# CouncilmanJeremyJamm/path_tracer

Measured on AMD Instinct MI355X. Metric: Mray/s at 1920x1080, 256 spp; achieved HBM GB/s in traversal kernel, higher is better.
Workload: dtype f32; 1 GPU; Cornell box (36 triangles, 6 BLAS) 1920x1080, 256 spp, depth 8, NEE+MIS; parallelism=rows/1, bvh_in_lds=True, scene_bytes=4208

## Files before the change

### path_tracer_amd/csrc/pt_api.cpp

```cpp
#include "../../include/pt_api.h"

#include <hip/hip_runtime.h>

#include <algorithm>
#include <chrono>
#include <cmath>
#include <cstdio>
#include <cstdlib>
#include <cstring>
#include <mutex>
#include <string>
#include <vector>

#include "pt_kernels.h"
#include "pt_png.h"
#include "pt_scene.h"

using namespace pt;

#ifndef PT_SHADE_BLOCKS_PER_CU
#define PT_SHADE_BLOCKS_PER_CU 16
#endif
#ifndef PT_JOIN_LATE
#define PT_JOIN_LATE 0
// ... 222 lines not shown
    if ((r = up(c->d_materials, f.materials.data(), f.materials.size() * sizeof(DMaterial)))) return r;
    if ((r = up(c->d_lights, f.lights.data(), f.lights.size() * sizeof(DLight)))) return r;

    SceneView& sv = c->sv;
    uint8_t* base = (uint8_t*)c->d_blob.p;
    sv.nodes = (const DNode*)base;
    sv.tri_isect = (const DTriIsect*)(base + nb);
    sv.instances = (const DInstance*)(base + nb + tb);
    sv.tri_shade = (const DTriVerts*)c->d_tri_shade.p;
    sv.tri_pos = (const DTriVerts*)c->d_tri_pos.p;
    sv.tri_orig = (const uint32_t*)c->d_tri_orig.p;
    sv.materials = (const DMaterial*)c->d_materials.p;
    sv.lights = (const DLight*)c->d_lights.p;
    sv.n_nodes = (uint32_t)f.nodes.size();
    sv.n_tris = (uint32_t)f.tri_isect.size();
    sv.n_instances = (uint32_t)f.instances.size();
    sv.n_materials = (uint32_t)f.materials.size();
    sv.n_lights = (uint32_t)f.lights.size();
    sv.world_root = f.world_root;
    sv.lights_root = f.lights_root;
    sv.prim_bits = f.prim_bits;
    sv.light_weight_sum = f.light_weight_sum;
    sv.blob_bytes = (uint32_t)blob.size();
    sv.stack_entries = f.stack_entries;
    sv.has_volumes = f.has_volumes ? 1u : 0u;
    c->ident_tlas = f.ident_tlas;

    c->lds_scene = blob.size() <= 48 * 1024 && !(c->cfg.flags & PT_FLAG_NO_LDS_SCENE);
    uint32_t threads = 256;
#ifndef PT_STACK_LDS_LEVELS
#define PT_STACK_LDS_LEVELS 14
#endif
    sv.stack_lds = std::min<uint32_t>(sv.stack_entries, c->cfg.stack_lds_levels ? c->cfg.stack_lds_levels : PT_STACK_LDS_LEVELS);
    auto lds_need = [&](uint32_t t) { return trace_lds_bytes(c->lds_scene, sv.blob_bytes, sv.stack_lds, t); };
    while (threads > 64 && lds_need(threads) > 64 * 1024) threads >>= 1;
    if (lds_need(threads) > 160 * 1024) return fail(c, PT_ERR_LIMIT, "BVH too deep for the LDS traversal stack");
    c->block_threads = threads;
    const size_t lds = lds_need(threads);
    uint32_t per_cu = (uint32_t)std::min<size_t>((160 * 1024) / std::max<size_t>(lds, 1), 2048 / threads);
    per_cu = std::max(1u, std::min(per_cu, (uint32_t)PT_TRACE_BLOCKS_PER_CU_MAX));
    c->trace_blocks = (uint32_t)c->n_cus * per_cu;
    sv.stack_spill = nullptr;
    if (sv.stack_entries > sv.stack_lds)
    {
        const size_t lanes = (size_t)c->trace_blocks * threads;
        c->spill_region_words = (size_t)(sv.stack_entries - sv.stack_lds) * lanes;
        if ((r = dev_alloc(c, c->d_spill, 2 * pt_ctx::kMaxPipes * c->spill_region_words * 8))) return r;
        sv.stack_spill = (uint64_t*)c->d_spill.p;
    }

    for (uint32_t q = 0; q < Q_COUNT; ++q) c->class_present[q] = (q == Q_TERMINAL);
    for (const DInstance& in : f.instances) c->class_present[in.qclass & 0xffu] = true;
    c->scene_uploaded = true;
    c->stats.scene_bytes = blob.size();
    c->stats.lds_scene = c->lds_scene;
    c->stats.stack_entries = sv.stack_entries;
    return PT_OK;
}

TraceLaunch trace_launch(pt_ctx* c, int pipe = 0, bool side_stream = false)
{
    TraceLaunch tl;
    tl.scene = c->sv;
    if (tl.scene.stack_spill) tl.scene.stack_spill += (size_t)(2 * pipe + (side_stream ? 1 : 0)) * c->spill_region_words;
    tl.blob = c->d_blob.p;
    tl.lds_scene = c->lds_scene;
    tl.ident_tlas = (c->cfg.flags & PT_FLAG_GENERAL_WALK) ? 0u : c->ident_tlas;
// ... 1967 lines not shown
```

### path_tracer_amd/csrc/pt_kernels.h

```cpp
#pragma once
#include <hip/hip_runtime.h>

#include "pt_materials.h"
#include "pt_types.h"

namespace pt {

struct TraceLaunch
{
    SceneView scene;
    const void* blob;
    bool lds_scene;
    uint32_t ident_tlas;
    uint32_t grid_blocks;
    uint32_t n_cus;
    uint32_t block_threads;
};

inline size_t trace_lds_bytes(bool lds_scene, uint32_t blob_bytes, uint32_t stack_lds, uint32_t block_threads)
{
    return (lds_scene ? (size_t)blob_bytes : 0) + (size_t)stack_lds * block_threads * 8;
}
inline size_t trace_lds_bytes(const TraceLaunch& tl) { return trace_lds_bytes(tl.lds_scene, tl.scene.blob_bytes, tl.scene.stack_lds, tl.block_threads); }

struct WavefrontBuffers
{
    PathState st;
    RayQueue rq[2];
    RayQueue rq_shadow;
    RayQueue rq_lchain[2];
    f4* lchain_nb[2];
    f4* lchain_hit;
    f4* hits;
    f4* q_shade_base;
    uint32_t q_stride;
    uint32_t q_class_slot;
    uint2* q_term[2];
    Counters* counters;
    uint32_t* heads;
    uint4* wave_times;
    uint4* wave_times_any;
    uint32_t* tails;
    uint32_t cap_slots;
    uint32_t cap_slots_shade;
    uint32_t cap_slots_term;
    uint32_t class_mask;
};

inline ShadeQueue shade_queue(const WavefrontBuffers& wb, uint32_t q)
{
    const size_t slot = (wb.q_class_slot >> (4u * q)) & 0xfu;
    f4* a = wb.q_shade_base + 3u * slot * (size_t)wb.q_stride;
    return ShadeQueue{a, a + wb.q_stride, a + 2u * (size_t)wb.q_stride};
}

void launch_generate(hipStream_t s, const RenderParams& rp, const CameraView& cam, const WavefrontBuffers& wb, const uint2* list = nullptr);
// ... 35 lines not shown
```

### path_tracer_amd/csrc/pt_kernels.hip

```cpp
#include "pt_kernels.h"
#include "pt_materials.h"

#include <algorithm>
#include <mutex>
#include <vector>

namespace pt {
namespace {

#ifndef PT_STEPS_PER_ROUND
#define PT_STEPS_PER_ROUND 8
#endif
#ifndef PT_REFILL_BELOW
#define PT_REFILL_BELOW 40
#endif
#ifndef PT_STEPS_PER_ROUND_GLOBAL_BVH
#define PT_STEPS_PER_ROUND_GLOBAL_BVH 4
#endif
#ifndef PT_REFILL_BELOW_GLOBAL_BVH
#define PT_REFILL_BELOW_GLOBAL_BVH 56
#endif
#ifndef PT_STEPS_ANY
#define PT_STEPS_ANY 4
#endif
// ... 366 lines not shown
            else base = nb;
        }
        sh.base[q] = base;
    }
    __syncthreads();
#pragma unroll
    for (int q = 0; q < 4; ++q) pos[q] = sh.base[q] + sh.wave_rank[q][wid] + mbcnt64(m[q]);
    __syncthreads();
}

__device__ __forceinline__ f3 xyz(const f4& v) { return f3{v.x, v.y, v.z}; }
__device__ __forceinline__ float asf(uint32_t u) { return __uint_as_float(u); }
__device__ __forceinline__ uint32_t asu(float f) { return __float_as_uint(f); }

typedef float nt4_t __attribute__((ext_vector_type(4)));
__device__ __forceinline__ void nt_store(f4* p, f4 v) { __builtin_nontemporal_store(nt4_t{v.x, v.y, v.z, v.w}, reinterpret_cast<nt4_t*>(p)); }
__device__ __forceinline__ f4 nt_load(const f4* p) { const nt4_t v = __builtin_nontemporal_load(reinterpret_cast<const nt4_t*>(p)); return f4{v.x, v.y, v.z, v.w}; }


__device__ __forceinline__ bool slab(const uint4 w0, const uint4 w1, const f3 o, const f3 inv, const float t_max, float& t_enter)
{
    const bool nx = inv.x < 0.0f, ny = inv.y < 0.0f, nz = inv.z < 0.0f;
    typedef float pair_t __attribute__((ext_vector_type(2)));
    const pair_t px = (pair_t{asf(nx ? w1.x : w0.x), asf(nx ? w0.x : w1.x)} - pair_t{o.x, o.x}) * pair_t{inv.x, inv.x};
    const pair_t py = (pair_t{asf(ny ? w1.y : w0.y), asf(ny ? w0.y : w1.y)} - pair_t{o.y, o.y}) * pair_t{inv.y, inv.y};
    const pair_t pz = (pair_t{asf(nz ? w1.z : w0.z), asf(nz ? w0.z : w1.z)} - pair_t{o.z, o.z}) * pair_t{inv.z, inv.z};
    const float tnx = px.x, tfx = px.y, tny = py.x, tfy = py.y, tnz = pz.x, tfz = pz.y;
    const float ts = fmaxf(fmaxf(fmaxf(tnx, tny), tnz), PT_EPSILON);
    const float tb = fminf(fminf(fminf(tfx, tfy), tfz), t_max);
    t_enter = ts;
    return ts <= tb;
}

__device__ __forceinline__ bool sign_differs(float a, float b)
{
    return __builtin_isunordered(a, b) || (((asu(a) ^ asu(b)) >> 31) != 0u);
}

__device__ __forceinline__ bool tri_planes(const uint4 p0, const uint4 p1, const uint4 p2, const f3 o, const f3 d, const float t_max,
                                           const float t_est, float& td, float& ud, float& vd, float& det)
{
    const f3 mo = fma3(d, bc3(t_est), o);
    const float t_min = PT_EPSILON - t_est, t_mx = t_max - t_est;
    const f4 n0{asf(p0.x), asf(p0.y), asf(p0.z), asf(p0.w)};
    det = dot3(d, xyz(n0));
    td = -dot4(f4{mo.x, mo.y, mo.z, -1.0f}, n0);
    const bool out_t = sign_differs(td - det * t_min, det * t_mx - td);
    const f3 p = det * mo + td * d;
    const f4 p4{p.x, p.y, p.z, det};
    ud = dot4(p4, f4{asf(p1.x), asf(p1.y), asf(p1.z), asf(p1.w)});
    const bool out_u = sign_differs(ud, det - ud);
    vd = dot4(p4, f4{asf(p2.x), asf(p2.y), asf(p2.z), asf(p2.w)});
    const bool out_v = sign_differs(vd, det - ud - vd);
    return !(out_t | out_u | out_v);
}

struct TriEval { float td, ud, vd, det; bool uv_ok; };
__device__ __forceinline__ TriEval tri_eval(const uint4* tp, const f3 mo, const f3 d)
{
    TriEval e;
    const uint4 p0 = tp[0], p1 = tp[1], p2 = tp[2];
    const f4 n0{asf(p0.x), asf(p0.y), asf(p0.z), asf(p0.w)};
    e.det = dot3(d, xyz(n0));
    e.td = -dot4(f4{mo.x, mo.y, mo.z, -1.0f}, n0);
    const f3 p = e.det * mo + e.td * d;
    const f4 p4{p.x, p.y, p.z, e.det};
    e.ud = dot4(p4, f4{asf(p1.x), asf(p1.y), asf(p1.z), asf(p1.w)});
    e.vd = dot4(p4, f4{asf(p2.x), asf(p2.y), asf(p2.z), asf(p2.w)});
    const bool out_u = sign_differs(e.ud, e.det - e.ud), out_v = sign_differs(e.vd, e.det - e.ud - e.vd);
    e.uv_ok = !out_u && !out_v;
    return e;
}
__device__ __forceinline__ bool tri_in_range(const TriEval& e, float t_min, float t_mx) { return !sign_differs(e.td - e.det * t_min, e.det * t_mx - e.td); }

struct Blob
{
    const uint4* nodes;
    const uint4* tris;
    const uint4* inst;
    const uint2* leaves;
};
__device__ __forceinline__ void leaf_range(const Blob& bl, uint32_t kind, uint32_t payload, uint32_t& first, uint32_t& count)
{
    if (kind == NODE_TRIS) { first = payload & LEAF_FIRST_MASK; count = (payload >> LEAF_FIRST_BITS) + 1u; }
    else { const uint2 lf = bl.leaves[payload]; first = lf.x; count = lf.y; }
}

struct LaneRay { f3 o, d, inv; };

__device__ __forceinline__ void pin(uint4& v) { asm volatile("" : "+v"(v.x), "+v"(v.y), "+v"(v.z), "+v"(v.w)); }
template <bool EAGER, bool ROOT_BOX>
__device__ __forceinline__ LaneRay to_object(const Blob& bl, uint32_t inst, const LaneRay& w, bool ray_finite, uint4& root0, uint4& root1)
{
    const uint4* ip = bl.inst + INST_WORDS * inst;
    uint4 r0, r1, r2;
    if (EAGER)
    {
        r0 = ip[0]; r1 = ip[1]; r2 = ip[2];
    }
    const uint4 meta = ip[INST_META_WORD];
    if (ROOT_BOX) { root0 = ip[INST_ROOT_WORD]; root1 = ip[INST_ROOT_WORD + 1u]; }
    else root0.w = reinterpret_cast<const uint32_t*>(ip + INST_ROOT_WORD)[3];
    if (EAGER) { pin(r0); pin(r1); pin(r2); }
    LaneRay r;
    if ((meta.w & INSTANCE_IDENTITY) != 0u && ray_finite)
    {
        const uint32_t so = asu(w.o.x) & asu(w.o.y) & asu(w.o.z) & 0x80000000u;
        const uint32_t sd = asu(w.d.x) & asu(w.d.y) & asu(w.d.z) & 0x80000000u;
        r.o.x = w.o.x != 0.0f ? w.o.x : asf(so);
        r.o.y = w.o.y != 0.0f ? w.o.y : asf(so);
        r.o.z = w.o.z != 0.0f ? w.o.z : asf(so);
        r.d.x = w.d.x != 0.0f ? w.d.x : asf(sd);
        r.d.y = w.d.y != 0.0f ? w.d.y : asf(sd);
        r.d.z = w.d.z != 0.0f ? w.d.z : asf(sd);
        r.inv.x = w.d.x != 0.0f ? w.inv.x : asf(sd | 0x7f800000u);
        r.inv.y = w.d.y != 0.0f ? w.inv.y : asf(sd | 0x7f800000u);
        r.inv.z = w.d.z != 0.0f ? w.inv.z : asf(sd | 0x7f800000u);
        return r;
    }
// ... 3 lines not shown
    r.o.z = ((asf(r2.x) * w.o.x + asf(r2.y) * w.o.y) + asf(r2.z) * w.o.z) + asf(r2.w);
    r.d.x = (asf(r0.x) * w.d.x + asf(r0.y) * w.d.y) + asf(r0.z) * w.d.z;
    r.d.y = (asf(r1.x) * w.d.x + asf(r1.y) * w.d.y) + asf(r1.z) * w.d.z;
    r.d.z = (asf(r2.x) * w.d.x + asf(r2.y) * w.d.y) + asf(r2.z) * w.d.z;
    r.inv = rcp3(r.d);
    return r;
}

__device__ __forceinline__ LaneRay ident_ray(const LaneRay& w)
{
    const uint32_t so = asu(w.o.x) & asu(w.o.y) & asu(w.o.z) & 0x80000000u;
    const uint32_t sd = asu(w.d.x) & asu(w.d.y) & asu(w.d.z) & 0x80000000u;
    LaneRay r;
    r.o.x = w.o.x != 0.0f ? w.o.x : asf(so);
    r.o.y = w.o.y != 0.0f ? w.o.y : asf(so);
    r.o.z = w.o.z != 0.0f ? w.o.z : asf(so);
    r.d.x = w.d.x != 0.0f ? w.d.x : asf(sd);
    r.d.y = w.d.y != 0.0f ? w.d.y : asf(sd);
    r.d.z = w.d.z != 0.0f ? w.d.z : asf(sd);
    r.inv = w.inv;
    return r;
}
__device__ __forceinline__ uint32_t ray_signs(const LaneRay& w)
{
    return (asu(w.o.x) >> 31) | ((asu(w.o.y) >> 31) << 1) | ((asu(w.o.z) >> 31) << 2) |
           ((asu(w.d.x) >> 31) << 3) | ((asu(w.d.y) >> 31) << 4) | ((asu(w.d.z) >> 31) << 5);
}
__device__ __forceinline__ f3 with_signs(const f3 v, uint32_t bits)
{
    return f3{asf((asu(v.x) & 0x7fffffffu) | ((bits & 1u) << 31)), asf((asu(v.y) & 0x7fffffffu) | (((bits >> 1) & 1u) << 31)),
              asf((asu(v.z) & 0x7fffffffu) | (((bits >> 2) & 1u) << 31))};
}

template <bool LDS_SCENE>
__device__ __forceinline__ Blob stage_scene(const SceneView& sv, const uint4* __restrict__ gblob, uint4* smem, uint32_t& words)
{
    Blob b;
    const uint4* base = gblob;
    words = 0;
    if (LDS_SCENE)
    {
        words = sv.blob_bytes >> 4;
        for (uint32_t i = threadIdx.x; i < words; i += blockDim.x) smem[i] = gblob[i];
        __syncthreads();
        base = smem;
    }
    b.nodes = base;
    b.tris = base + 2u * sv.n_nodes;
    b.inst = base + 2u * sv.n_nodes + 3u * sv.n_tris;
    b.leaves = reinterpret_cast<const uint2*>(base + 2u * sv.n_nodes + 3u * sv.n_tris + INST_WORDS * sv.n_instances);
    return b;
}

enum { CLOSEST_WORLD = 0, CLOSEST_LIGHTS = 1, CLOSEST_HOOK = 2, CLOSEST_PRIMARY = 3 };

struct ClosestOut
{
    f4* hits;
    f4* q_base;
    uint32_t q_stride, q_class_slot;
    uint2* q_term;
    uint32_t* n_shade;
    uint4* wave_times;
    uint32_t* tails;
    uint32_t cap_shade, cap_term;
    uint32_t class_mask;
    uint32_t* overflow;
    uint32_t world_root;
    uint8_t* occl;
    f3 eye;
    f4* radiance;
    f4* first_pos;
    uint32_t* first_id;
    uint32_t keep_s_id, keep_s_pos, blk_log, n_blk, blk_last, act_pixels;
    FastDiv div_blk_paths, div_blk_last;
    uint32_t finalize_miss;
    const DPathRec* rec;
    uint32_t enable_nee;
};

template <bool SPILL>
struct Stack8;
template <>
// ... 229 lines not shown
            if (!active && rank < take)
            {
                const uint32_t mine = first + rank;
                const f4 b = rb[mine];
                ray_idx = mine;
                pid = asu(b.w);
                if (pid != HOLE) {
                valid_rays += 1u;
                if (MODE == CLOSEST_PRIMARY)
                {
                    w.o = f3{out->eye.x, out->eye.y, out->eye.z};
                    t_max = asf(0x7f800000u);
                }
                else
                {
                    const f4 a = ra[mine];
                    w.o = xyz(a);
                    t_max = a.w;
                }
                w.d = xyz(b);
                w.inv = rcp3(w.d);
                ray_finite = finite3(w.o) && finite3(w.d);
                if (IDENT) { ob = ident_ray(w); w_signs = ray_signs(w); }
                bid = MISS_ID;
                any_phase = false;
                chain_code = 2u;
                bt = asf(0x7f800000u);
                hud = 0.0f;
                hvd = 0.0f;
                hdet = 1.0f;
                in_blas = false;
                sp = stk.empty();
                float te;
                const uint4 root0 = bl.nodes[2u * root];
                const bool ok = (t_max == t_max) && (!IDENT || ray_finite) && slab(root0, bl.nodes[2u * root + 1u], IDENT ? ob.o : w.o, w.inv, t_max, te);
                if (ok)
                {
                    stk.put(sp, make_uint2(root0.w, 0u));
                    sp = stk.up(sp);
                    active = true;
                }
                else { pending = true; }
                }
            }
#if PT_WAVE_TIMES
            if (tw_first == 0u && take != 0u) tw_first = (uint32_t)wall_clock64() | 1u;
#endif
            act = __ballot(active);
            if (act == 0ull) continue;
            if (PT_RESERVICE && take < (uint32_t)__popcll(idle) && !wr.drained && (uint32_t)__popcll(act) <= (uint32_t)Refill<LDS_SCENE>::kBelow) continue;
        }

#pragma unroll 1
        for (int it = 0; it < Refill<LDS_SCENE>::kSteps; ++it)
        {
#if PT_STEP_STATS
            {
                const uint64_t am = __ballot(active);
                if (am != 0ull) { st_iter += 1u; st_lane_active += (uint32_t)__popcll(am); }
            }
#endif
            if (!active) continue;
            if (!IDENT && in_blas && sp == blas_base) in_blas = false;
            if (MODE == CLOSEST_LIGHTS && any_phase)
            {
                if (sp == stk.empty()) { active = false; pending = true; chain_code = 0u; continue; }
                sp = stk.down(sp);
                const uint2 e = stk.get(sp);
                uint32_t link = e.x;
                float t_enter = asf(e.y);
                if ((link >> NODE_KIND_SHIFT) == NODE_INSTANCE)
                {
                    uint4 r0, r1;
                    if (IDENT)
                    {
                        const uint4* ip = bl.inst + INST_WORDS * (link & NODE_PAYLOAD_MASK) + INST_ROOT_WORD;
                        r0 = ip[0]; r1 = ip[1];
                    }
                    else
                    {
                        ob = to_object<!LDS_SCENE, true>(bl, link & NODE_PAYLOAD_MASK, w, ray_finite, r0, r1);
                        in_blas = true;
                        blas_base = sp;
                    }
                    if (!slab(r0, r1, ob.o, ob.inv, t_max, t_enter)) continue;
                    link = r0.w;
                }
                const uint32_t kkind = link >> NODE_KIND_SHIFT, kpay = link & NODE_PAYLOAD_MASK;
                if (kkind == NODE_BRANCH)
                {
                    const uint4* cp = bl.nodes + 2u * kpay;
                    const uint4 l0 = cp[0], l1 = cp[1], r0 = cp[2], r1 = cp[3];
                    const f3 so = (IDENT || in_blas) ? ob.o : w.o, sinv = (IDENT || in_blas) ? ob.inv : w.inv;
                    float tl, tr;
                    const bool hl = slab(l0, l1, so, sinv, t_max, tl);
                    const bool hr = slab(r0, r1, so, sinv, t_max, tr);
                    if (hl) { stk.put(sp, make_uint2(l0.w, asu(tl))); sp = stk.up(sp); }
                    if (hr) { stk.put(sp, make_uint2(r0.w, asu(tr))); sp = stk.up(sp); }
                }
                else
                {
                    uint32_t first, count;
                    leaf_range(bl, kkind, kpay, first, count);
                    for (uint32_t k = 0; k < count; ++k)
                    {
                        const uint4* tp = bl.tris + 3u * (first + k);
                        float td, ud, vd, det;
                        if (tri_planes(tp[0], tp[1], tp[2], ob.o, ob.d, t_max, t_enter, td, ud, vd, det))
                        {
                            active = false;
                            pending = true;
                            chain_code = 1u;
                            break;
                        }
                    }
                }
                continue;
            }
            if (sp == stk.empty())
            {
                if (MODE == CLOSEST_LIGHTS && bid != MISS_ID)
                {
                    light_hits += 1u;
                    any_phase = true;
                    in_blas = false;
                    t_max = bt * (1.0f - PT_EPSILON);
                    float te = 0.0f;
                    const uint4 wr0 = bl.nodes[2u * lights_world_root];
                    if (t_max == t_max && slab(wr0, bl.nodes[2u * lights_world_root + 1u], IDENT ? ob.o : w.o, IDENT ? ob.inv : w.inv, t_max, te)) { stk.put(sp, make_uint2(wr0.w, asu(te))); sp = stk.up(sp); }
                    else { active = false; pending = true; chain_code = 0u; }
                    continue;
                }
                active = false;
                pending = true;
                continue;
            }
            sp = stk.down(sp);
            const uint2 e = stk.get(sp);
            if (asf(e.y) > t_max) continue;
            uint32_t link = e.x;
            float t_est = asf(e.y);
#if PT_STEP_STATS
            { const bool x = (link >> NODE_KIND_SHIFT) == NODE_INSTANCE; const uint64_t m = __ballot(x); st_lane_inst += x ? 1u : 0u; if (m != 0ull && lane_id() == (uint32_t)__builtin_ctzll(m)) st_wave_inst += 1u; }
#endif
            if ((link >> NODE_KIND_SHIFT) == NODE_INSTANCE)
            {
                uint4 root0, root1;
                inst = link & NODE_PAYLOAD_MASK;
                if (IDENT) root0.w = reinterpret_cast<const uint32_t*>(bl.inst + INST_WORDS * inst + INST_ROOT_WORD)[3];
                else
                {
                    ob = to_object<!LDS_SCENE, false>(bl, inst, w, ray_finite, root0, root1);
                    in_blas = true;
                    blas_base = sp;
                }
                if (0.0f > t_max) continue;
                link = root0.w;
                t_est = 0.0f;
            }
            uint32_t kind = link >> NODE_KIND_SHIFT, payload = link & NODE_PAYLOAD_MASK;
#if PT_STEP_STATS
            { const bool x = kind == NODE_BRANCH; const uint64_t m = __ballot(x); st_lane_branch += x ? 1u : 0u; if (m != 0ull && lane_id() == (uint32_t)__builtin_ctzll(m)) st_wave_branch += 1u; }
#endif
#pragma unroll 1
            for (int lvl = 0; lvl < PT_BRANCH_LEVELS && kind == NODE_BRANCH; ++lvl)
            {
                const uint4* cp = bl.nodes + 2u * payload;
                const uint4 l0 = cp[0], l1 = cp[1], r0 = cp[2], r1 = cp[3];
                const f3 o = (IDENT || in_blas) ? ob.o : w.o, inv = (IDENT || in_blas) ? ob.inv : w.inv;
                float tl, tr;
                const bool hl = slab(l0, l1, o, inv, t_max, tl);
                const bool hr = slab(r0, r1, o, inv, t_max, tr);
                const bool left_near = tl < tr;
                const uint2 le = make_uint2(l0.w, asu(tl)), re = make_uint2(r0.w, asu(tr));
                if (hl && hr) { stk.put(sp, left_near ? re : le); sp = stk.up(sp); }
                kind = NODE_INSTANCE;
                if (hl || hr)
                {
                    const uint2 near = (hl && (left_near || !hr)) ? le : re;
                    const uint32_t nk = near.x >> NODE_KIND_SHIFT;
                    if ((nk & 1u) != 0u || (nk == NODE_BRANCH && lvl + 1 < PT_BRANCH_LEVELS))
                    {
                        kind = nk;
                        payload = near.x & NODE_PAYLOAD_MASK;
                        t_est = asf(near.y);
                    }
                    else { stk.put(sp, near); sp = stk.up(sp); }
                }
            }
#if PT_STEP_STATS
            { const bool x = (kind & 1u) != 0u; const uint64_t m = __ballot(x); st_lane_leaf += x ? 1u : 0u; if (m != 0ull && lane_id() == (uint32_t)__builtin_ctzll(m)) st_wave_leaf += 1u; }
#endif
            if (kind & 1u)
            {
                uint32_t first, count;
                leaf_range(bl, kind, payload, first, count);
                const f3 mo = fma3(ob.d, bc3(t_est), ob.o);
                const float t_min = PT_EPSILON - t_est;
                auto accept = [&](const TriEval& e, uint32_t tri) {
                    if (e.uv_ok && tri_in_range(e, t_min, t_max - t_est))
                    {
                        bt = e.td / e.det + t_est;
                        hud = e.ud;
                        hvd = e.vd;
                        hdet = e.det;
                        t_max = bt;
                        bid = (inst << prim_bits) | tri;
// ... 105 lines not shown
    for (;;)
    {
        uint64_t act = __ballot(active);
        const bool no_more = wr.drained && wr.cur >= wr.end;
#if PT_WAVE_TIMES
        if (no_more && tw_drained == 0u) tw_drained = (uint32_t)wall_clock64() | 1u;
#endif
        const bool service = no_more ? (act == 0ull) : (__popcll(act) <= Refill<LDS_SCENE>::kBelowAny);
        if (service)
        {
            if (no_more) break;
            const uint64_t idle = ~act;
            uint32_t first;
            const uint32_t take = claim_rays(wr, heads, plan, (uint32_t)__popcll(idle), first);
            const uint32_t rank = mbcnt64(idle);
            if (!active && rank < take)
            {
                const uint32_t mine = first + rank;
                const f4 a = ra[mine], b = rb[mine];
                const uint32_t tag = asu(b.w);
                if (tag != HOLE) {
                valid_rays += 1u;
                path_ends = MODE == ANY_SHADOW && (tag & PATH_ENDS) != 0u;
                out_idx = (MODE == ANY_HOOK) ? mine : (tag & ~PATH_ENDS);
                w.o = xyz(a);
                w.d = xyz(b);
                w.inv = rcp3(w.d);
                ray_finite = finite3(w.o) && finite3(w.d);
                if (IDENT) ob = ident_ray(w);
                t_max = a.w;
                in_blas = false;
                sp = stk.empty();
                float te;
                const uint4 root0 = bl.nodes[2u * root];
                const bool ok = (t_max == t_max) && (!IDENT || ray_finite) && slab(root0, bl.nodes[2u * root + 1u], IDENT ? ob.o : w.o, w.inv, t_max, te);
                if (ok)
                {
                    stk.put(sp, make_uint2(root0.w, asu(te)));
                    sp = stk.up(sp);
                    active = true;
                }
                else put_result(0u);
                }
            }
            act = __ballot(active);
            if (act == 0ull) continue;
            if (PT_RESERVICE && take < (uint32_t)__popcll(idle) && !wr.drained && (uint32_t)__popcll(act) <= (uint32_t)Refill<LDS_SCENE>::kBelowAny) continue;
        }

#pragma unroll 1
        for (int it = 0; it < Refill<LDS_SCENE>::kStepsAny; ++it)
        {
#if PT_STEP_STATS
            {
                const uint64_t am = __ballot(active);
                if (am != 0ull) { st_iter += 1u; st_lane_active += (uint32_t)__popcll(am); }
            }
#endif
            if (!active) continue;
            if (!IDENT && in_blas && sp == blas_base) in_blas = false;
            if (sp == stk.empty())
            {
                active = false;
                put_result(0u);
                continue;
            }
            sp = stk.down(sp);
            const uint2 e = stk.get(sp);
            uint32_t link = e.x;
            float t_enter = asf(e.y);
#if PT_STEP_STATS
            { const bool x = (link >> NODE_KIND_SHIFT) == NODE_INSTANCE; const uint64_t m = __ballot(x); st_lane_inst += x ? 1u : 0u; if (m != 0ull && lane_id() == (uint32_t)__builtin_ctzll(m)) st_wave_inst += 1u; }
#endif
            if ((link >> NODE_KIND_SHIFT) == NODE_INSTANCE)
            {
                uint4 r0, r1;
                if (IDENT)
                {
                    const uint4* ip = bl.inst + INST_WORDS * (link & NODE_PAYLOAD_MASK) + INST_ROOT_WORD;
                    r0 = ip[0]; r1 = ip[1];
                }
                else
                {
                    ob = to_object<!LDS_SCENE, true>(bl, link & NODE_PAYLOAD_MASK, w, ray_finite, r0, r1);
                    in_blas = true;
                    blas_base = sp;
                }
                if (!slab(r0, r1, ob.o, ob.inv, t_max, t_enter)) continue;
                link = r0.w;
            }
            uint32_t kind = link >> NODE_KIND_SHIFT, payload = link & NODE_PAYLOAD_MASK;
#if PT_STEP_STATS
            { const bool x = kind == NODE_BRANCH; const uint64_t m = __ballot(x); st_lane_branch += x ? 1u : 0u; if (m != 0ull && lane_id() == (uint32_t)__builtin_ctzll(m)) st_wave_branch += 1u; }
#endif
#pragma unroll 1
            for (int lvl = 0; lvl < PT_BRANCH_LEVELS_ANY && kind == NODE_BRANCH; ++lvl)
            {
                const uint4* cp = bl.nodes + 2u * payload;
                const uint4 l0 = cp[0], l1 = cp[1], r0 = cp[2], r1 = cp[3];
                const f3 o = (IDENT || in_blas) ? ob.o : w.o, inv = (IDENT || in_blas) ? ob.inv : w.inv;
                float tl, tr;
                const bool hl = slab(l0, l1, o, inv, t_max, tl);
                const bool hr = slab(r0, r1, o, inv, t_max, tr);
                if (hl && hr) { stk.put(sp, make_uint2(l0.w, asu(tl))); sp = stk.up(sp); }
                kind = NODE_INSTANCE;
                if (hl || hr)
                {
                    const uint2 next = hr ? make_uint2(r0.w, asu(tr)) : make_uint2(l0.w, asu(tl));
                    const uint32_t nk = next.x >> NODE_KIND_SHIFT;
                    if ((nk & 1u) != 0u || (nk == NODE_BRANCH && lvl + 1 < PT_BRANCH_LEVELS_ANY))
                    {
                        kind = nk;
                        payload = next.x & NODE_PAYLOAD_MASK;
                        t_enter = asf(next.y);
                    }
                    else { stk.put(sp, next); sp = stk.up(sp); }
                }
            }
#if PT_STEP_STATS
            { const bool x = (kind & 1u) != 0u; const uint64_t m = __ballot(x); st_lane_leaf += x ? 1u : 0u; if (m != 0ull && lane_id() == (uint32_t)__builtin_ctzll(m)) st_wave_leaf += 1u; }
#endif
            if (kind & 1u)
            {
                uint32_t first, count;
                leaf_range(bl, kind, payload, first, count);
                for (uint32_t k = 0; k < count; ++k)
                {
                    const uint4* tp = bl.tris + 3u * (first + k);
                    float td, ud, vd, det;
                    if (tri_planes(tp[0], tp[1], tp[2], ob.o, ob.d, t_max, t_enter, td, ud, vd, det))
                    {
                        active = false;
                        put_result(1u);
                        break;
                    }
                }
            }
        }
    }
#if PT_STEP_STATS
    if (MODE == ANY_SHADOW)
// ... 281 lines not shown
                {
                    const PidParts pp = pid_split(rp, pid);
                    if (pp.s == rp.keep_s_pos)
                    {
                        const f3 p = fma3(xyz(rb), bc3(hit.x), xyz(ra));
                        io.st.first_pos[pp.k] = f4{p.x, p.y, p.z, hit.x};
                    }
                    if (pp.s >= rp.keep_s_id) io.st.first_id[(pp.s - rp.keep_s_id) * rp.act_pixels + pp.k] = in.blas & 0xffu;
                }
                const DMaterial& m = sv.materials[in.material];
                if (!rp.enable_nee || (flags & FLAG_LAST_DELTA) || bounce == 0u)
                    acc = fma3(f3{m.colour[0], m.colour[1], m.colour[2]}, pw, acc);
            }
        }
        io.st.radiance[pid] = f4{acc.x, acc.y, acc.z, 0.0f};
    }
}

template <bool IDENT>
__device__ __forceinline__ bool inline_any(const Blob& bl, const Stack8<false>& stk, const uint32_t root, const f4 ra, const f4 rb, const bool want)
{
    bool active = false, blocked = false, in_blas = false, ray_finite = false;
    LaneRay w{}, ob{};
    const float t_max = ra.w;
    uint32_t sp = stk.empty(), blas_base = 0u;
    if (want)
    {
        w.o = xyz(ra);
        w.d = xyz(rb);
        w.inv = rcp3(w.d);
        ray_finite = finite3(w.o) && finite3(w.d);
        if (IDENT) ob = ident_ray(w);
        float te;
        const uint4 root0 = bl.nodes[2u * root];
        if ((t_max == t_max) && (!IDENT || ray_finite) && slab(root0, bl.nodes[2u * root + 1u], IDENT ? ob.o : w.o, w.inv, t_max, te))
        {
            stk.put(sp, make_uint2(root0.w, asu(te)));
            sp = stk.up(sp);
            active = true;
        }
    }
    while (__ballot(active) != 0ull)
    {
        if (!active) continue;
        if (!IDENT && in_blas && sp == blas_base) in_blas = false;
        if (sp == stk.empty()) { active = false; continue; }
        sp = stk.down(sp);
        const uint2 e = stk.get(sp);
        uint32_t link = e.x;
        float t_enter = asf(e.y);
        if ((link >> NODE_KIND_SHIFT) == NODE_INSTANCE)
        {
            uint4 r0, r1;
            if (IDENT)
            {
                const uint4* ip = bl.inst + INST_WORDS * (link & NODE_PAYLOAD_MASK) + INST_ROOT_WORD;
                r0 = ip[0]; r1 = ip[1];
            }
            else
            {
                ob = to_object<false, true>(bl, link & NODE_PAYLOAD_MASK, w, ray_finite, r0, r1);
                in_blas = true;
                blas_base = sp;
            }
            if (!slab(r0, r1, ob.o, ob.inv, t_max, t_enter)) continue;
            link = r0.w;
        }
        uint32_t kind = link >> NODE_KIND_SHIFT, payload = link & NODE_PAYLOAD_MASK;
#pragma unroll 1
        for (int lvl = 0; lvl < PT_BRANCH_LEVELS_INLINE && kind == NODE_BRANCH; ++lvl)
        {
            const uint4* cp = bl.nodes + 2u * payload;
            const uint4 l0 = cp[0], l1 = cp[1], r0 = cp[2], r1 = cp[3];
            const f3 o = (IDENT || in_blas) ? ob.o : w.o, inv = (IDENT || in_blas) ? ob.inv : w.inv;
            float tl, tr;
            const bool hl = slab(l0, l1, o, inv, t_max, tl);
            const bool hr = slab(r0, r1, o, inv, t_max, tr);
            if (hl && hr) { stk.put(sp, make_uint2(l0.w, asu(tl))); sp = stk.up(sp); }
            kind = NODE_INSTANCE;
            if (hl || hr)
            {
                const uint2 next = hr ? make_uint2(r0.w, asu(tr)) : make_uint2(l0.w, asu(tl));
                const uint32_t nk = next.x >> NODE_KIND_SHIFT;
                if ((nk & 1u) != 0u || (nk == NODE_BRANCH && lvl + 1 < PT_BRANCH_LEVELS_INLINE))
                {
                    kind = nk;
                    payload = next.x & NODE_PAYLOAD_MASK;
                    t_enter = asf(next.y);
                }
                else { stk.put(sp, next); sp = stk.up(sp); }
            }
        }
        if (kind & 1u)
        {
            uint32_t first, count;
            leaf_range(bl, kind, payload, first, count);
            for (uint32_t k = 0; k < count; ++k)
            {
                const uint4* tp = bl.tris + 3u * (first + k);
                float td, ud, vd, det;
                if (tri_planes(tp[0], tp[1], tp[2], ob.o, ob.d, t_max, t_enter, td, ud, vd, det))
                {
                    active = false;
                    blocked = true;
                    break;
                }
            }
        }
    }
    return blocked;
}

struct ShadeKArgs { SceneView sv; RenderParams rp; ShadeIO io; uint32_t bounce; const uint4* gblob; uint32_t world_root; };
typedef const __attribute__((address_space(4))) ShadeKArgs* ShadeKArgsPtr;
__device__ __forceinline__ const ShadeKArgs& shade_args()
// ... 286 lines not shown
        if (want_lchain) { io.rq_lchain.a[pos[1]] = lc_a; io.rq_lchain.b[pos[1]] = lc_b; io.lchain_nb[pos[1]] = nee_b; nee_e.w = asf(pos[1]); }
        if (want_next) { nt_store(io.rq_out.a + pos[2], nx_a); nt_store(io.rq_out.b + pos[2], nx_b); }
        if (want_dead) io.q_term_next[pos[3]] = make_uint2(pid | ENTRY_DEAD, pid);
        const bool write_rec = valid && (want_next || want_dead || ends_with_shadow);
        if (valid && !write_rec) io.st.radiance[pid] = f4{acc.x, acc.y, acc.z, 0.0f};
        {
            float m[4][4] = {{pw.x, pw.y, pw.z, asf(draws)}, {acc.x, acc.y, acc.z, asf(flags)}, {nee_e.x, nee_e.y, nee_e.z, nee_e.w}, {nee_pw.x, nee_pw.y, nee_pw.z, nee_pw.w}};
            const uint32_t q = threadIdx.x & 3u;
#pragma unroll
            for (int c = 0; c < 4; ++c)
            {
                float a0 = m[0][c], a1 = m[1][c], a2 = m[2][c], a3 = m[3][c];
                { const float t = (q & 1u) ? a0 : a1; const float r = asf(__builtin_amdgcn_mov_dpp(asu(t), 0xB1, 0xF, 0xF, true)); if (q & 1u) a0 = r; else a1 = r; }
                { const float t = (q & 1u) ? a2 : a3; const float r = asf(__builtin_amdgcn_mov_dpp(asu(t), 0xB1, 0xF, 0xF, true)); if (q & 1u) a2 = r; else a3 = r; }
                { const float t = (q & 2u) ? a0 : a2; const float r = asf(__builtin_amdgcn_mov_dpp(asu(t), 0x4E, 0xF, 0xF, true)); if (q & 2u) a0 = r; else a2 = r; }
                { const float t = (q & 2u) ? a1 : a3; const float r = asf(__builtin_amdgcn_mov_dpp(asu(t), 0x4E, 0xF, 0xF, true)); if (q & 2u) a1 = r; else a3 = r; }
                m[0][c] = a0; m[1][c] = a1; m[2][c] = a2; m[3][c] = a3;
            }
            const uint32_t wr = write_rec ? 1u : 0u;
#define PT_QUAD_STORE(K, SEL)                                                                                                   \
            {                                                                                                                      \
                const uint32_t pid_k = __builtin_amdgcn_mov_dpp(pid, SEL, 0xF, 0xF, true);                \
                const uint32_t wr_k = __builtin_amdgcn_mov_dpp(wr, SEL, 0xF, 0xF, true);                                           \
                if (wr_k != 0u) reinterpret_cast<f4*>(io.st.rec + pid_k)[q] = f4{m[K][0], m[K][1], m[K][2], m[K][3]};             \
            }
            PT_QUAD_STORE(0, 0x00) PT_QUAD_STORE(1, 0x55) PT_QUAD_STORE(2, 0xAA) PT_QUAD_STORE(3, 0xFF)
#undef PT_QUAD_STORE
        }
        if (INLINE)
        {
            uint32_t tid = threadIdx.x;
            asm volatile("" : "+v"(tid));
            const ShadeKArgs& ka2 = shade_args();
            const uint32_t blob_words = ka2.sv.blob_bytes >> 4;
            Blob bl;
            bl.nodes = smem_dyn;
            bl.tris = smem_dyn + 2u * ka2.sv.n_nodes;
            bl.inst = smem_dyn + 2u * ka2.sv.n_nodes + 3u * ka2.sv.n_tris;
            bl.leaves = reinterpret_cast<const uint2*>(smem_dyn + 2u * ka2.sv.n_nodes + 3u * ka2.sv.n_tris + INST_WORDS * ka2.sv.n_instances);
            const Stack8<false> stk{reinterpret_cast<char*>(smem_dyn), blob_words * 16u + tid * 8u, blockDim.x * 8u};
            traced += (uint32_t)__popcll(__ballot(want_shadow));
            culled += (uint32_t)__popcll(__ballot(cull_now));
            const bool blocked = inline_any<IDENT>(bl, stk, ka2.world_root, sh_a, sh_b, want_shadow);
            if (want_shadow)
            {
                DPathRec* rec = shade_args().io.st.rec + pid;
                if (ends_with_shadow)
                {
                    const f3 e = blocked ? f3{0.0f, 0.0f, 0.0f} : xyz(rec->nee_e);
                    const f3 a2 = xyz(rec->acc) + xyz(rec->nee_pw) * (e + f3{0.0f, 0.0f, 0.0f});
                    shade_args().io.st.radiance[pid] = f4{a2.x, a2.y, a2.z, 0.0f};
                }
                else if (blocked)
                {
                    float* e = reinterpret_cast<float*>(&rec->nee_e);
                    e[0] = 0.0f; e[1] = 0.0f; e[2] = 0.0f;
                }
            }
            a_next = (idx + stride) < n ? nt_load(shade_args().io.q_in.a + idx + stride) : hole_a;
        }
    }
    if (!INLINE) add_tally(io.lchain_heads, culled, HEAD_TALLY2);
    else if (lane_id() == 0u)
    {
        const uint32_t wave = blockIdx.x * (blockDim.x >> 6) + (threadIdx.x >> 6);
        const uint32_t line = ((wave * 7u) & (kQueueHeads - 1u)) * kHeadStrideWords;
        if (culled != 0u) atomicAdd(io.lchain_heads + line + HEAD_TALLY2, culled);
        if (traced != 0u) atomicAdd(io.shadow_heads + line + HEAD_TALLY0, traced);
    }
}

#undef PT_SHADE_ARGS
// ... 630 lines not shown
```

Measured before the change: 14730 Mray/s.

## Repack LDS BVH nodes into sign-indexed slab records for branchless child tests

When the scene is staged in LDS, BVH nodes are rewritten into a 10-dword record per node laid out as (min,max,min) triplets per axis plus a link word. The ray's direction sign picks an offset into each triplet, so near/far slab values are read directly and no min/max swap is needed per axis. The goal is fewer ALU ops and narrower LDS reads per child test. In exchange LDS staging gets more complex, node storage grows from 8 to 10 dwords, and accesses become scalar dword loads instead of 128-bit loads, which could add LDS instructions.

Result: faster. 14940 Mray/s, median of 6 (+1.4%).

```diff
diff --git a/path_tracer_amd/csrc/pt_api.cpp b/path_tracer_amd/csrc/pt_api.cpp
--- a/path_tracer_amd/csrc/pt_api.cpp
+++ b/path_tracer_amd/csrc/pt_api.cpp
@@ -278,7 +278,7 @@
 #define PT_STACK_LDS_LEVELS 14
 #endif
     sv.stack_lds = std::min<uint32_t>(sv.stack_entries, c->cfg.stack_lds_levels ? c->cfg.stack_lds_levels : PT_STACK_LDS_LEVELS);
-    auto lds_need = [&](uint32_t t) { return trace_lds_bytes(c->lds_scene, sv.blob_bytes, sv.stack_lds, t); };
+    auto lds_need = [&](uint32_t t) { return trace_lds_bytes(c->lds_scene, sv.blob_bytes, sv.n_nodes, sv.stack_lds, t); };
     while (threads > 64 && lds_need(threads) > 64 * 1024) threads >>= 1;
     if (lds_need(threads) > 160 * 1024) return fail(c, PT_ERR_LIMIT, "BVH too deep for the LDS traversal stack");
     c->block_threads = threads;
diff --git a/path_tracer_amd/csrc/pt_kernels.h b/path_tracer_amd/csrc/pt_kernels.h
--- a/path_tracer_amd/csrc/pt_kernels.h
+++ b/path_tracer_amd/csrc/pt_kernels.h
@@ -17,11 +17,15 @@
     uint32_t block_threads;
 };
 
-inline size_t trace_lds_bytes(bool lds_scene, uint32_t blob_bytes, uint32_t stack_lds, uint32_t block_threads)
+enum : uint32_t { LDS_NODE_DWORDS = 10u, LDS_NODE_LINK = 9u };
+__host__ __device__ inline uint32_t lds_node_words(uint32_t n_nodes) { return (n_nodes * LDS_NODE_DWORDS * 4u + 15u) >> 4; }
+__host__ __device__ inline uint32_t lds_blob_bytes(uint32_t blob_bytes, uint32_t n_nodes) { return blob_bytes - n_nodes * (uint32_t)sizeof(DNode) + lds_node_words(n_nodes) * 16u; }
+
+inline size_t trace_lds_bytes(bool lds_scene, uint32_t blob_bytes, uint32_t n_nodes, uint32_t stack_lds, uint32_t block_threads)
 {
-    return (lds_scene ? (size_t)blob_bytes : 0) + (size_t)stack_lds * block_threads * 8;
+    return (lds_scene ? (size_t)lds_blob_bytes(blob_bytes, n_nodes) : 0) + (size_t)stack_lds * block_threads * 8;
 }
-inline size_t trace_lds_bytes(const TraceLaunch& tl) { return trace_lds_bytes(tl.lds_scene, tl.scene.blob_bytes, tl.scene.stack_lds, tl.block_threads); }
+inline size_t trace_lds_bytes(const TraceLaunch& tl) { return trace_lds_bytes(tl.lds_scene, tl.scene.blob_bytes, tl.scene.n_nodes, tl.scene.stack_lds, tl.block_threads); }
 
 struct WavefrontBuffers
 {
diff --git a/path_tracer_amd/csrc/pt_kernels.hip b/path_tracer_amd/csrc/pt_kernels.hip
--- a/path_tracer_amd/csrc/pt_kernels.hip
+++ b/path_tracer_amd/csrc/pt_kernels.hip
@@ -422,6 +422,25 @@
     return ts <= tb;
 }
 
+struct SlabOff { uint32_t x, y, z; };
+__device__ __forceinline__ SlabOff slab_off(const f3 inv) { return SlabOff{inv.x < 0.0f ? 4u : 0u, inv.y < 0.0f ? 4u : 0u, inv.z < 0.0f ? 4u : 0u}; }
+__device__ __forceinline__ bool slab_lds(const uint32_t* rec, const SlabOff so, const f3 o, const f3 inv, const float t_max, float& t_enter)
+{
+    const char* r = reinterpret_cast<const char*>(rec);
+    const float* ax = reinterpret_cast<const float*>(r + so.x);
+    const float* ay = reinterpret_cast<const float*>(r + so.y) + 3;
+    const float* az = reinterpret_cast<const float*>(r + so.z) + 6;
+    typedef float pair_t __attribute__((ext_vector_type(2)));
+    const pair_t px = (pair_t{ax[0], ax[1]} - pair_t{o.x, o.x}) * pair_t{inv.x, inv.x};
+    const pair_t py = (pair_t{ay[0], ay[1]} - pair_t{o.y, o.y}) * pair_t{inv.y, inv.y};
+    const pair_t pz = (pair_t{az[0], az[1]} - pair_t{o.z, o.z}) * pair_t{inv.z, inv.z};
+    const float tnx = px.x, tfx = px.y, tny = py.x, tfy = py.y, tnz = pz.x, tfz = pz.y;
+    const float ts = fmaxf(fmaxf(fmaxf(tnx, tny), tnz), PT_EPSILON);
+    const float tb = fminf(fminf(fminf(tfx, tfy), tfz), t_max);
+    t_enter = ts;
+    return ts <= tb;
+}
+
 __device__ __forceinline__ bool sign_differs(float a, float b)
 {
     return __builtin_isunordered(a, b) || (((asu(a) ^ asu(b)) >> 31) != 0u);
@@ -466,6 +485,7 @@
 struct Blob
 {
     const uint4* nodes;
+    const uint32_t* lnodes;
     const uint4* tris;
     const uint4* inst;
     const uint2* leaves;
@@ -475,6 +495,31 @@
     if (kind == NODE_TRIS) { first = payload & LEAF_FIRST_MASK; count = (payload >> LEAF_FIRST_BITS) + 1u; }
     else { const uint2 lf = bl.leaves[payload]; first = lf.x; count = lf.y; }
 }
+template <bool LDS_SCENE>
+__device__ __forceinline__ void test_children(const Blob& bl, const uint32_t payload, const f3 o, const f3 inv, const float t_max,
+                                              bool& hl, bool& hr, float& tl, float& tr, uint32_t& ll, uint32_t& lr)
+{
+    if (LDS_SCENE)
+    {
+        const uint32_t* rec = reinterpret_cast<const uint32_t*>(reinterpret_cast<const char*>(bl.lnodes) + __umul24(payload, LDS_NODE_DWORDS * 4u));
+        const SlabOff so = slab_off(inv);
+        hl = slab_lds(rec, so, o, inv, t_max, tl);
+        hr = slab_lds(rec + LDS_NODE_DWORDS, so, o, inv, t_max, tr);
+        ll = rec[LDS_NODE_LINK];
+        lr = rec[LDS_NODE_DWORDS + LDS_NODE_LINK];
+    }
+    else
+    {
+        const uint4* cp = bl.nodes + 2u * payload;
+        const uint4 l0 = cp[0], l1 = cp[1], r0 = cp[2], r1 = cp[3];
+        hl = slab(l0, l1, o, inv, t_max, tl);
+        hr = slab(r0, r1, o, inv, t_max, tr);
+        ll = l0.w;
+        lr = r0.w;
+    }
+}
+__device__ __forceinline__ uint4 lds_box0(const Blob& bl, uint32_t i) { const uint32_t* r = bl.lnodes + LDS_NODE_DWORDS * i; return make_uint4(r[0], r[3], r[6], r[LDS_NODE_LINK]); }
+__device__ __forceinline__ uint4 lds_box1(const Blob& bl, uint32_t i) { const uint32_t* r = bl.lnodes + LDS_NODE_DWORDS * i; return make_uint4(r[1], r[4], r[7], 0u); }
 
 struct LaneRay { f3 o, d, inv; };
 
@@ -544,23 +589,46 @@
               asf((asu(v.z) & 0x7fffffffu) | (((bits >> 2) & 1u) << 31))};
 }
 
+__device__ __forceinline__ Blob lds_blob(uint4* smem, uint32_t blob_bytes, uint32_t n_nodes, uint32_t n_tris, uint32_t n_instances, uint32_t& words)
+{
+    const uint32_t nw = lds_node_words(n_nodes);
+    Blob b;
+    b.nodes = nullptr;
+    b.lnodes = reinterpret_cast<const uint32_t*>(smem);
+    b.tris = smem + nw;
+    b.inst = smem + nw + 3u * n_tris;
+    b.leaves = reinterpret_cast<const uint2*>(smem + nw + 3u * n_tris + INST_WORDS * n_instances);
+    words = nw + (blob_bytes >> 4) - 2u * n_nodes;
+    return b;
+}
 template <bool LDS_SCENE>
 __device__ __forceinline__ Blob stage_scene(const SceneView& sv, const uint4* __restrict__ gblob, uint4* smem, uint32_t& words)
 {
     Blob b;
-    const uint4* base = gblob;
     words = 0;
     if (LDS_SCENE)
     {
-        words = sv.blob_bytes >> 4;
-        for (uint32_t i = threadIdx.x; i < words; i += blockDim.x) smem[i] = gblob[i];
+        b = lds_blob(smem, sv.blob_bytes, sv.n_nodes, sv.n_tris, sv.n_instances, words);
+        const uint32_t nw = lds_node_words(sv.n_nodes), rest = (sv.blob_bytes >> 4) - 2u * sv.n_nodes;
+        for (uint32_t i = threadIdx.x; i < rest; i += blockDim.x) smem[nw + i] = gblob[2u * sv.n_nodes + i];
+        uint32_t* rec = reinterpret_cast<uint32_t*>(smem);
+        for (uint32_t i = threadIdx.x; i < sv.n_nodes; i += blockDim.x)
+        {
+            const uint4 a = gblob[2u * i], m = gblob[2u * i + 1u];
+            uint32_t* r = rec + LDS_NODE_DWORDS * i;
+            r[0] = a.x; r[1] = m.x; r[2] = a.x;
+            r[3] = a.y; r[4] = m.y; r[5] = a.y;
+            r[6] = a.z; r[7] = m.z; r[8] = a.z;
+            r[LDS_NODE_LINK] = a.w;
+        }
         __syncthreads();
-        base = smem;
-    }
-    b.nodes = base;
-    b.tris = base + 2u * sv.n_nodes;
-    b.inst = base + 2u * sv.n_nodes + 3u * sv.n_tris;
-    b.leaves = reinterpret_cast<const uint2*>(base + 2u * sv.n_nodes + 3u * sv.n_tris + INST_WORDS * sv.n_instances);
+        return b;
+    }
+    b.nodes = gblob;
+    b.lnodes = nullptr;
+    b.tris = gblob + 2u * sv.n_nodes;
+    b.inst = gblob + 2u * sv.n_nodes + 3u * sv.n_tris;
+    b.leaves = reinterpret_cast<const uint2*>(gblob + 2u * sv.n_nodes + 3u * sv.n_tris + INST_WORDS * sv.n_instances);
     return b;
 }
 
@@ -856,8 +924,8 @@
                 in_blas = false;
                 sp = stk.empty();
                 float te;
-                const uint4 root0 = bl.nodes[2u * root];
-                const bool ok = (t_max == t_max) && (!IDENT || ray_finite) && slab(root0, bl.nodes[2u * root + 1u], IDENT ? ob.o : w.o, w.inv, t_max, te);
+                const uint4 root0 = LDS_SCENE ? lds_box0(bl, root) : bl.nodes[2u * root];
+                const bool ok = (t_max == t_max) && (!IDENT || ray_finite) && slab(root0, LDS_SCENE ? lds_box1(bl, root) : bl.nodes[2u * root + 1u], IDENT ? ob.o : w.o, w.inv, t_max, te);
                 if (ok)
                 {
                     stk.put(sp, make_uint2(root0.w, 0u));
@@ -913,14 +981,13 @@
                 const uint32_t kkind = link >> NODE_KIND_SHIFT, kpay = link & NODE_PAYLOAD_MASK;
                 if (kkind == NODE_BRANCH)
                 {
-                    const uint4* cp = bl.nodes + 2u * kpay;
-                    const uint4 l0 = cp[0], l1 = cp[1], r0 = cp[2], r1 = cp[3];
                     const f3 so = (IDENT || in_blas) ? ob.o : w.o, sinv = (IDENT || in_blas) ? ob.inv : w.inv;
                     float tl, tr;
-                    const bool hl = slab(l0, l1, so, sinv, t_max, tl);
-                    const bool hr = slab(r0, r1, so, sinv, t_max, tr);
-                    if (hl) { stk.put(sp, make_uint2(l0.w, asu(tl))); sp = stk.up(sp); }
-                    if (hr) { stk.put(sp, make_uint2(r0.w, asu(tr))); sp = stk.up(sp); }
+                    bool hl, hr;
+                    uint32_t ll, lr;
+                    test_children<LDS_SCENE>(bl, kpay, so, sinv, t_max, hl, hr, tl, tr, ll, lr);
+                    if (hl) { stk.put(sp, make_uint2(ll, asu(tl))); sp = stk.up(sp); }
+                    if (hr) { stk.put(sp, make_uint2(lr, asu(tr))); sp = stk.up(sp); }
                 }
                 else
                 {
@@ -950,8 +1017,8 @@
                     in_blas = false;
                     t_max = bt * (1.0f - PT_EPSILON);
                     float te = 0.0f;
-                    const uint4 wr0 = bl.nodes[2u * lights_world_root];
-                    if (t_max == t_max && slab(wr0, bl.nodes[2u * lights_world_root + 1u], IDENT ? ob.o : w.o, IDENT ? ob.inv : w.inv, t_max, te)) { stk.put(sp, make_uint2(wr0.w, asu(te))); sp = stk.up(sp); }
+                    const uint4 wr0 = LDS_SCENE ? lds_box0(bl, lights_world_root) : bl.nodes[2u * lights_world_root];
+                    if (t_max == t_max && slab(wr0, LDS_SCENE ? lds_box1(bl, lights_world_root) : bl.nodes[2u * lights_world_root + 1u], IDENT ? ob.o : w.o, IDENT ? ob.inv : w.inv, t_max, te)) { stk.put(sp, make_uint2(wr0.w, asu(te))); sp = stk.up(sp); }
                     else { active = false; pending = true; chain_code = 0u; }
                     continue;
                 }
@@ -989,14 +1056,13 @@
 #pragma unroll 1
             for (int lvl = 0; lvl < PT_BRANCH_LEVELS && kind == NODE_BRANCH; ++lvl)
             {
-                const uint4* cp = bl.nodes + 2u * payload;
-                const uint4 l0 = cp[0], l1 = cp[1], r0 = cp[2], r1 = cp[3];
                 const f3 o = (IDENT || in_blas) ? ob.o : w.o, inv = (IDENT || in_blas) ? ob.inv : w.inv;
                 float tl, tr;
-                const bool hl = slab(l0, l1, o, inv, t_max, tl);
-                const bool hr = slab(r0, r1, o, inv, t_max, tr);
+                bool hl, hr;
+                uint32_t ll, lr;
+                test_children<LDS_SCENE>(bl, payload, o, inv, t_max, hl, hr, tl, tr, ll, lr);
                 const bool left_near = tl < tr;
-                const uint2 le = make_uint2(l0.w, asu(tl)), re = make_uint2(r0.w, asu(tr));
+                const uint2 le = make_uint2(ll, asu(tl)), re = make_uint2(lr, asu(tr));
                 if (hl && hr) { stk.put(sp, left_near ? re : le); sp = stk.up(sp); }
                 kind = NODE_INSTANCE;
                 if (hl || hr)
@@ -1168,8 +1234,8 @@
                 in_blas = false;
                 sp = stk.empty();
                 float te;
-                const uint4 root0 = bl.nodes[2u * root];
-                const bool ok = (t_max == t_max) && (!IDENT || ray_finite) && slab(root0, bl.nodes[2u * root + 1u], IDENT ? ob.o : w.o, w.inv, t_max, te);
+                const uint4 root0 = LDS_SCENE ? lds_box0(bl, root) : bl.nodes[2u * root];
+                const bool ok = (t_max == t_max) && (!IDENT || ray_finite) && slab(root0, LDS_SCENE ? lds_box1(bl, root) : bl.nodes[2u * root + 1u], IDENT ? ob.o : w.o, w.inv, t_max, te);
                 if (ok)
                 {
                     stk.put(sp, make_uint2(root0.w, asu(te)));
@@ -1232,17 +1298,16 @@
 #pragma unroll 1
             for (int lvl = 0; lvl < PT_BRANCH_LEVELS_ANY && kind == NODE_BRANCH; ++lvl)
             {
-                const uint4* cp = bl.nodes + 2u * payload;
-                const uint4 l0 = cp[0], l1 = cp[1], r0 = cp[2], r1 = cp[3];
                 const f3 o = (IDENT || in_blas) ? ob.o : w.o, inv = (IDENT || in_blas) ? ob.inv : w.inv;
                 float tl, tr;
-                const bool hl = slab(l0, l1, o, inv, t_max, tl);
-                const bool hr = slab(r0, r1, o, inv, t_max, tr);
-                if (hl && hr) { stk.put(sp, make_uint2(l0.w, asu(tl))); sp = stk.up(sp); }
+                bool hl, hr;
+                uint32_t ll, lr;
+                test_children<LDS_SCENE>(bl, payload, o, inv, t_max, hl, hr, tl, tr, ll, lr);
+                if (hl && hr) { stk.put(sp, make_uint2(ll, asu(tl))); sp = stk.up(sp); }
                 kind = NODE_INSTANCE;
                 if (hl || hr)
                 {
-                    const uint2 next = hr ? make_uint2(r0.w, asu(tr)) : make_uint2(l0.w, asu(tl));
+                    const uint2 next = hr ? make_uint2(lr, asu(tr)) : make_uint2(ll, asu(tl));
                     const uint32_t nk = next.x >> NODE_KIND_SHIFT;
                     if ((nk & 1u) != 0u || (nk == NODE_BRANCH && lvl + 1 < PT_BRANCH_LEVELS_ANY))
                     {
@@ -1590,8 +1655,8 @@
         ray_finite = finite3(w.o) && finite3(w.d);
         if (IDENT) ob = ident_ray(w);
         float te;
-        const uint4 root0 = bl.nodes[2u * root];
-        if ((t_max == t_max) && (!IDENT || ray_finite) && slab(root0, bl.nodes[2u * root + 1u], IDENT ? ob.o : w.o, w.inv, t_max, te))
+        const uint4 root0 = lds_box0(bl, root);
+        if ((t_max == t_max) && (!IDENT || ray_finite) && slab(root0, lds_box1(bl, root), IDENT ? ob.o : w.o, w.inv, t_max, te))
         {
             stk.put(sp, make_uint2(root0.w, asu(te)));
             sp = stk.up(sp);
@@ -1628,17 +1693,16 @@
 #pragma unroll 1
         for (int lvl = 0; lvl < PT_BRANCH_LEVELS_INLINE && kind == NODE_BRANCH; ++lvl)
         {
-            const uint4* cp = bl.nodes + 2u * payload;
-            const uint4 l0 = cp[0], l1 = cp[1], r0 = cp[2], r1 = cp[3];
             const f3 o = (IDENT || in_blas) ? ob.o : w.o, inv = (IDENT || in_blas) ? ob.inv : w.inv;
             float tl, tr;
-            const bool hl = slab(l0, l1, o, inv, t_max, tl);
-            const bool hr = slab(r0, r1, o, inv, t_max, tr);
-            if (hl && hr) { stk.put(sp, make_uint2(l0.w, asu(tl))); sp = stk.up(sp); }
+            bool hl, hr;
+            uint32_t ll, lr;
+            test_children<true>(bl, payload, o, inv, t_max, hl, hr, tl, tr, ll, lr);
+            if (hl && hr) { stk.put(sp, make_uint2(ll, asu(tl))); sp = stk.up(sp); }
             kind = NODE_INSTANCE;
             if (hl || hr)
             {
-                const uint2 next = hr ? make_uint2(r0.w, asu(tr)) : make_uint2(l0.w, asu(tl));
+                const uint2 next = hr ? make_uint2(lr, asu(tr)) : make_uint2(ll, asu(tl));
                 const uint32_t nk = next.x >> NODE_KIND_SHIFT;
                 if ((nk & 1u) != 0u || (nk == NODE_BRANCH && lvl + 1 < PT_BRANCH_LEVELS_INLINE))
                 {
@@ -1991,12 +2055,8 @@
             uint32_t tid = threadIdx.x;
             asm volatile("" : "+v"(tid));
             const ShadeKArgs& ka2 = shade_args();
-            const uint32_t blob_words = ka2.sv.blob_bytes >> 4;
-            Blob bl;
-            bl.nodes = smem_dyn;
-            bl.tris = smem_dyn + 2u * ka2.sv.n_nodes;
-            bl.inst = smem_dyn + 2u * ka2.sv.n_nodes + 3u * ka2.sv.n_tris;
-            bl.leaves = reinterpret_cast<const uint2*>(smem_dyn + 2u * ka2.sv.n_nodes + 3u * ka2.sv.n_tris + INST_WORDS * ka2.sv.n_instances);
+            uint32_t blob_words;
+            const Blob bl = lds_blob(smem_dyn, ka2.sv.blob_bytes, ka2.sv.n_nodes, ka2.sv.n_tris, ka2.sv.n_instances, blob_words);
             const Stack8<false> stk{reinterpret_cast<char*>(smem_dyn), blob_words * 16u + tid * 8u, blockDim.x * 8u};
             traced += (uint32_t)__popcll(__ballot(want_shadow));
             culled += (uint32_t)__popcll(__ballot(cull_now));
```
